# saidwivedi/InteractVLM

Measured on AMD Instinct MI355X. Metric: images/sec end-to-end contact inference, higher is better.
Workload: dtype f16

## Files before the change

### include/ivlm_hip.h

```cpp
#ifndef IVLM_HIP_H
#define IVLM_HIP_H

#include <stddef.h>
#include <stdint.h>

#ifdef __cplusplus
extern "C" {
#endif

#define IVLM_OK 0
#define IVLM_ERR_INVALID_ARG (-1)
#define IVLM_ERR_WORKSPACE (-2)
#define IVLM_ERR_LAUNCH (-3)
#define IVLM_ERR_UNSUPPORTED (-4)

#define IVLM_F32 0
#define IVLM_BF16 1
#define IVLM_BF16_SPLIT 2
#define IVLM_F16 4
#define IVLM_F16_SPLIT 5
#define IVLM_FP8 3

#define IVLM_GEMM_A_F32 1
#define IVLM_GEMM_RES_F32 2
// ... 233 lines not shown
typedef struct {
    int embed_dim, depth, heads, grid, window, patch, img_size, out_chans, mlp_dim;
} ivlm_sam_cfg;
typedef struct {
    const void *patch_w, *patch_b, *pos_embed, *neck0_w, *neck1_w, *neck1_b, *neck2_w, *neck3_w, *neck3_b;
} ivlm_sam_head;
typedef struct {
    const void *norm1_w, *norm1_b, *qkv_w, *qkv_b, *rel_h, *rel_w, *rel_cat, *proj_w, *proj_b, *norm2_w, *norm2_b, *lin1_w, *lin1_b,
        *lin2_w, *lin2_b;
    int global_attn;
} ivlm_sam_block;
size_t ivlm_sam_encode_workspace_bytes(const ivlm_sam_cfg *cfg, int V);
int ivlm_sam_encode(const ivlm_sam_cfg *cfg, const ivlm_sam_head *head, const ivlm_sam_block *blocks_host, const void *images, int V,
                    float *embeddings_out, void *workspace, size_t workspace_bytes, ivlm_stream_t stream);
size_t ivlm_sam_encode_parity_workspace_bytes(const ivlm_sam_cfg *cfg, int V);
int ivlm_sam_encode_parity(const ivlm_sam_cfg *cfg, const ivlm_sam_head *head, const ivlm_sam_block *blocks_host, const void *images,
                           int V, float *embeddings_out, void *workspace, size_t workspace_bytes, ivlm_stream_t stream);
typedef struct {
    const void *lin1_w16, *lin2_w16;
} ivlm_sam_mlp_f16;
int ivlm_sam_encode_parity_f16mlp(const ivlm_sam_cfg *cfg, const ivlm_sam_head *head, const ivlm_sam_block *blocks_host,
                                  const ivlm_sam_mlp_f16 *mlp16_host, const void *images, int V, float *embeddings_out,
                                  void *workspace, size_t workspace_bytes, ivlm_stream_t stream);
typedef struct {
    const void *qkv_w16, *proj_w16, *lin1_w16, *lin2_w16, *qkv_b16, *rel_cat16;
} ivlm_sam_block_f16;
size_t ivlm_sam_encode_f16_workspace_bytes(const ivlm_sam_cfg *cfg, int V);
int ivlm_sam_encode_f16(const ivlm_sam_cfg *cfg, const ivlm_sam_head *head, const ivlm_sam_block *blocks_host,
                        const ivlm_sam_block_f16 *blocks16_host, const void *images, int V, float *embeddings_out, void *workspace,
                        size_t workspace_bytes, ivlm_stream_t stream);
int ivlm_bf16_to_f16(const void *src_bf16, void *dst_f16, int64_t n, ivlm_stream_t stream);

typedef struct {
    const void *w2, *b;
    int n, k;
} ivlm_lin;
typedef struct {
    ivlm_lin q, k, v, o;
} ivlm_dec_attn;
typedef struct {
    ivlm_dec_attn self_attn, t2i, i2t;
    const void *norm1_w, *norm1_b, *norm2_w, *norm2_b, *norm3_w, *norm3_b, *norm4_w, *norm4_b;
    ivlm_lin lin1, lin2;
} ivlm_dec_layer;
typedef struct {
    int C, heads, depth;
    const void *no_mask, *key_pe, *out_tokens;
    ivlm_dec_layer layers[4];
    ivlm_dec_attn final_attn;
    const void *norm_final_w, *norm_final_b, *up_ln_w, *up_ln_b;
    ivlm_lin up0, up1, hyper[3], iou[3];
} ivlm_sam_dec;
size_t ivlm_sam_decode_workspace_bytes(int V, int grid, int C, int n_text, int mlp_dim);
int ivlm_sam_decode(const ivlm_sam_dec *weights, int V, int grid, int n_text, const float *image_embeddings,
                    const float *text_embeds, float *low_res_out, float *iou_out, void *workspace, size_t workspace_bytes,
                    ivlm_stream_t stream);

int ivlm_gemm_splitk_choice(int M, int N, int K, int act, int has_rms);
int ivlm_stages_splitk_fused(int on);

int ivlm_gemv1_bf12(const float *x, const void *P, int64_t ldp, const void *E, int64_t lde, const int32_t *ebase,
                    const int32_t *patch_ptr, const int32_t *patch_col, const void *patch_val, void *C, const void *bias,
                    const void *residual, int N, int K, int act, int out_f32, const void *rms_w, float rms_eps, int flags,
                    ivlm_stream_t stream);
int ivlm_gemv1_bf12m(const float *x, const void *Pf, const void *Ef, const int32_t *ebase, const int32_t *patch_ptr,
                     const int32_t *patch_col, const void *patch_val, void *C, const void *bias, const void *residual, int N, int K,
                     int act, int out_f32, const void *rms_w, float rms_eps, int flags, ivlm_stream_t stream);
int ivlm_llama_decode_attn_parts(const float *qkv, int cache_dtype, void *kcache, void *vcache, int tmax, float *parts, int H, int D,
                                 int pos, const int32_t *pos_dev, float theta, float scale, const float *cos_tab, const float *sin_tab,
                                 ivlm_stream_t stream);
int ivlm_gemv1_bf12m_parts(const float *parts, int D, const void *Pf, const void *Ef, const int32_t *ebase, const int32_t *patch_ptr,
                           const int32_t *patch_col, const void *patch_val, void *C, const void *bias, const void *residual, int N, int K,
                           int act, int out_f32, int flags, ivlm_stream_t stream);
int ivlm_pack_bf12m_count(const void *w, int N_valid, int n_rows, int K, int32_t *ebase, int32_t *patch_ptr, ivlm_stream_t stream);
int ivlm_pack_bf12m_fill(const void *w, int N_valid, int n_rows, int K, const int32_t *ebase, const int32_t *patch_ptr, void *Pf, void *Ef,
                         int32_t *patch_col, void *patch_val, ivlm_stream_t stream);
int ivlm_gemv16_bf12m(const float *x, int64_t lda, int M, const void *Pf, const void *Ef, const int32_t *ebase,
                      const int32_t *patch_ptr, const int32_t *patch_col, const void *patch_val, void *C, int64_t ldc, const void *bias,
                      const void *residual, int64_t ldr, int N, int K, int act, int out_f32, const void *rms_w, float rms_eps, int flags,
                      ivlm_stream_t stream);
void ivlm_gemv16_bf12m_tuning(int tiles_per_block);
int ivlm_decode_parts_tuning(int ranges);
void ivlm_gemv1_bf12m_tuning(int wide_max_blocks);
int ivlm_unpack_bf12(const void *P, int64_t ldp, const void *E, int64_t lde, const int32_t *ebase, const int32_t *patch_ptr,
                     const int32_t *patch_col, const void *patch_val, int N, int K, void *w_out, ivlm_stream_t stream);

int ivlm_argmax_f32(const float *x, int rows, int cols, int32_t *out, ivlm_stream_t stream);
int ivlm_argmax_f32_bump(const float *x, int rows, int cols, int32_t *out, int32_t *bump, ivlm_stream_t stream);

int ivlm_im2col_nchw(const void *x, void *out, int B, int C, int H, int W, int ks, int stride, int Kpad,
                     ivlm_stream_t stream);
int ivlm_im2col3x3_nhwc(const void *x, void *out, int B, int H, int W, int C, ivlm_stream_t stream);
int ivlm_im2col3x3_nhwc_strided(const void *x, int64_t ldx, void *out, int64_t ldo, int B, int H, int W, int C,
                                ivlm_stream_t stream);
int ivlm_gather_rows(void *dst, int dst_kind, int64_t ldd, const void *src, int src_dtype, int64_t lds, const int32_t *idx,
                     const void *add, int add_dtype, int64_t lda, int64_t rows, int cols, const float *fp8_scale,
                     ivlm_stream_t stream);
int ivlm_amax(const void *x, int dtype, int64_t n, float *out, ivlm_stream_t stream);
int ivlm_add_rows(void *out, int out_kind, const void *a, int a_dtype, const void *b, int b_dtype, int64_t rows, int cols,
                  int64_t b_rows, int op, ivlm_stream_t stream);
int ivlm_fill_rows(void *dst, int64_t ldd, const int32_t *idx, int64_t n_idx, const void *row, int cols,
                   ivlm_stream_t stream);
int ivlm_dense_pe(const void *gauss, void *pe, int pe_dtype, int h, int w, int F, ivlm_stream_t stream);
int ivlm_rope_kv(void *qkv, int64_t ld, int T, int H, int D, int pos0, float theta, void *kcache, void *vcache,
                 const float *cos_tab, const float *sin_tab, ivlm_stream_t stream);
int ivlm_rope_kv_f16(void *qkv, int64_t ld, int T, int H, int D, int pos0, float theta, void *kcache, void *vcache,
                     const float *cos_tab, const float *sin_tab, ivlm_stream_t stream);
int ivlm_rope_kv_split(void *qkv, int64_t ld, int T, int H, int D, int pos0, void *kcache, void *kcache_lo, void *vcache,
                       void *vcache_lo, const float *cos_tab, const float *sin_tab, ivlm_stream_t stream);
int ivlm_llama_attn_oproj(const float *qkv, void *kcache, void *vcache, int tmax, float *attn_scratch, const void *wo,
                          const float *x, float *x_out, int H, int D, float theta, float scale, const float *cos_tab,
                          const float *sin_tab, const int32_t *pos_dev, const int32_t *step_dev, int32_t *counter,
                          int32_t *status, ivlm_stream_t stream);
int ivlm_rope_table(float *cos_tab, float *sin_tab, int T, int D, float theta, ivlm_stream_t stream);
int ivlm_normalize_pad_u8(const uint8_t *src, int H, int W, int y0, int x0, int ch, int cw, const float *mean3_host,
                          const float *std3_host, void *out, int out_bf16, int OH, int OW, ivlm_stream_t stream);
int ivlm_mask_dot(const void *up, const void *hyper, int dtype, float *low, int B, int gh, int gw, int C,
                  ivlm_stream_t stream);

size_t ivlm_h_geo_workspace_bytes(int n);
int ivlm_h_geo_metric(const float *dist, const float *pred, const float *gt, int B, int n, float *out, void *workspace,
                      size_t workspace_bytes, ivlm_stream_t stream);
int ivlm_contact_prf(const float *gt, const float *pred, int B, int n, float thr, float *out, ivlm_stream_t stream);
int ivlm_spmv_csr(const int32_t *row_ptr, const int32_t *col, const float *val, const float *x, int B, int rows,
                  int cols, float *y, ivlm_stream_t stream);

int ivlm_contact_band_census(const float *p, int64_t ld, int B, int Nv, const float *thr, int J, float margin, int32_t *counts,
                             float *mindist, ivlm_stream_t stream);
size_t ivlm_mask_band_census_workspace_bytes(void);
int ivlm_mask_band_census(const float *logits, int V, int64_t HW, const int32_t *ent_pix, const int32_t *row_ptr, int n_rows,
                          float thr_p, float margin_p, int32_t *counts, void *workspace, size_t workspace_bytes,
                          ivlm_stream_t stream);

#define IVLM_SEG_GT_U8 0
#define IVLM_SEG_GT_I32 1
#define IVLM_SEG_GT_F32 2
size_t ivlm_seg_iou_workspace_bytes(int V);
int ivlm_seg_iou_counts(const float *pred, const void *gt, int gt_dtype, int V, int H, int W, int ignore_label, int32_t *out,
                        void *workspace, size_t workspace_bytes, ivlm_stream_t stream);
#define IVLM_AFFORD_MAX_N 4096
#define IVLM_AFFORD_MAX_T 64
int ivlm_afford_metrics(const float *gt, const float *pred, int B, int n, const float *thresholds, int T, float mae_div,
                        float *out, int32_t *valid, ivlm_stream_t stream);

#define IVLM_CONTACT_PAIR_CHAIN 512
size_t ivlm_contact_pair_workspace_bytes(int B, int N_o, int N_h);
int ivlm_contact_pair(const float *o, const float *h, const void *p, const void *q, int p_dtype, int B, int N_o, int N_h,
                      int64_t o_batch_stride, int64_t h_batch_stride, float *value_out, float *grad_o, float *grad_h,
                      void *workspace, size_t workspace_bytes, ivlm_stream_t stream);

#define IVLM_ICP_ESTIMATE_SCALE 1
#define IVLM_ICP_ALLOW_REFLECTION 2
#define IVLM_ICP_REQUERY 4
size_t ivlm_contact_icp_workspace_bytes(int B, int N_o);
int ivlm_contact_icp(const float *x, const float *y, const float *xn, const float *yn, const float *w, const float *init_R,
                     const float *init_T, const float *init_s, int B, int N_o, int N_h, int64_t x_batch_stride, int64_t y_batch_stride,
                     int64_t xn_batch_stride, int64_t yn_batch_stride, int64_t w_batch_stride, int max_iterations, float relative_rmse_thr,
                     int flags, float *R_out, float *T_out, float *s_out, float *rmse_out, int32_t *converged_out, int32_t *iterations_out,
                     int32_t *nn_idx_out, float *hist_R, float *hist_T, float *hist_s, void *workspace, size_t workspace_bytes,
                     ivlm_stream_t stream);

int ivlm_points_align(const float *X, const float *Y, const float *w, int B, int N, int64_t x_batch_stride, int64_t y_batch_stride,
                      int64_t w_batch_stride, int flags, float *R_out, float *T_out, float *s_out, void *workspace, size_t workspace_bytes,
                      ivlm_stream_t stream);

int ivlm_contact_nearest(const float *q, const float *t, int D, int B, int N_o, int N_h, int64_t q_batch_stride, int64_t t_batch_stride,
// ... 20 lines not shown
```

### interactvlm_amd/csrc/gemv_p12.hip

```cpp
#include <algorithm>

#include "kernels.h"

namespace ivlm {
namespace {

typedef __attribute__((ext_vector_type(4))) unsigned int u32x4_t;
typedef __attribute__((ext_vector_type(2))) unsigned int u32x2_t;
typedef __attribute__((ext_vector_type(4))) float f32x4v_t;

constexpr int kWaves = 16;
constexpr int kXScaleExp = 64;

struct P12 {
    const uint8_t* P;
    const uint8_t* E;
    int64_t ldp, lde;
    const int32_t* ebase;
    const int32_t* patch_ptr;
    const int32_t* patch_col;
    const bf16_t* patch_val;
};

template <int K>
// ... 69 lines not shown
        ssq = wave_sum(ssq);
        if (lane == 0) s_red[wave] = ssq;
    }
    __syncthreads();
    float acc = 0.0f;
    for (int c = lane; c < nw16; c += 64 * U) {
        if (c != lane) {
#pragma unroll
            for (int u = 0; u < U; ++u)
                if (c + 64 * u < nw16) {
                    w[u] = __builtin_nontemporal_load(pp + c + 64 * u);
                    e[u] = __builtin_nontemporal_load(ep + c + 64 * u);
                }
        }
#pragma unroll
        for (int u = 0; u < U; ++u) {
            const int cc = c + 64 * u;
            if (cc < nw16) {
                acc = dot4_p12(w[u][0], e[u][0], xf[2 * cc], acc);
                acc = dot4_p12(w[u][1], e[u][0] >> 16, xf[nchunk + 2 * cc], acc);
                acc = dot4_p12(w[u][2], e[u][1], xf[2 * cc + 1], acc);
                acc = dot4_p12(w[u][3], e[u][1] >> 16, xf[nchunk + 2 * cc + 1], acc);
            }
        }
    }
    float pacc = 0.0f;
    for (int i = p0 + lane; i < p1; i += 64) {
        const int col = p.patch_col[i];
        const int ch = col >> 3, wi = col & 7;
        const float xv = reinterpret_cast<const float*>(xf)[((wi < 4 ? ch : nchunk + ch) << 2) + (wi & 3)];
        pacc = fmaf(bf16_to_f32(p.patch_val[i]), xv, pacc);
    }
    acc = __builtin_ldexpf(wave_sum(acc), eb - kXScaleExp) + __builtin_ldexpf(wave_sum(pacc), -kXScaleExp);
    if (RMS) {
        float q = 0.0f;
#pragma unroll
        for (int i = 0; i < kWaves; ++i) q += s_red[i];
        acc *= rsqrtf(q / (float)g.K + g.rms_eps);
    }
    float v = acc + ((g.bias && live) ? bf16_to_f32(g.bias[row]) : 0.0f);
    if (g.act == ACT_SWIGLU) {
        if (lane == 0) s_val[wave] = v;
        __syncthreads();
        if (lane != 0 || (wave & 1) || !live) return;
        const float o = (v / (1.0f + __expf(-v))) * s_val[wave + 1];
        const int64_t idx = row >> 1;
        if (g.out_f32) static_cast<float*>(g.C)[idx] = o;
        else static_cast<bf16_t*>(g.C)[idx] = f32_to_bf16(o);
        return;
    }
    if (lane != 0 || !live) return;
    v = act1(v, g.act);
    if (g.residual) v += g.res_f32 ? reinterpret_cast<const float*>(g.residual)[row] : bf16_to_f32(g.residual[row]);
    if (g.out_f32) static_cast<float*>(g.C)[row] = v;
    else static_cast<bf16_t*>(g.C)[row] = f32_to_bf16(v);
}

struct P12M {
    const u32x4_t* P;
    const u32x2_t* E;
    const int32_t* ebase;
    const int32_t* patch_ptr;
    const int32_t* patch_col;
    const bf16_t* patch_val;
    const float* parts;
    int pD, pS;
};

typedef __attribute__((ext_vector_type(8))) __bf16 bf16x8m_t;
typedef __attribute__((ext_vector_type(4))) float f32x4m_t;

__device__ __forceinline__ uint32_t pair_p12m(uint32_t pd, uint32_t e) {
    return (pd & 0x807f807fu) | ((e * 0x00080080u) & 0x07800780u);
}
__device__ __forceinline__ bf16x8m_t frag_p12m(uint32_t x0, uint32_t x1, uint32_t e) {
    u32x4_t d;
    d[0] = pair_p12m(__builtin_amdgcn_perm(0u, x0, 0x01010000u), e & 0xffu);
    d[1] = pair_p12m(__builtin_amdgcn_perm(0u, x0, 0x03030202u), (e >> 8) & 0xffu);
    d[2] = pair_p12m(__builtin_amdgcn_perm(0u, x1, 0x01010000u), (e >> 16) & 0xffu);
    d[3] = pair_p12m(__builtin_amdgcn_perm(0u, x1, 0x03030202u), e >> 24);
    return __builtin_bit_cast(bf16x8m_t, d);
}

template <bool RMS, int kWavesM, int U, bool PARTS = false>
__global__ __launch_bounds__(64 * kWavesM, kWavesM == 16 ? 4 : 6) void gemv1_p12m_kernel(GemmArgs g, P12M p) {
    extern __shared__ __attribute__((aligned(16))) unsigned char smem[];
    __shared__ float s_red[kWavesM];
    __shared__ float s_part[kWavesM][16];
    __shared__ float s_patch[16];
    const int lane = threadIdx.x & 63, wave = __builtin_amdgcn_readfirstlane(threadIdx.x >> 6);
    const int K = g.K, nsp = K >> 6;
    const int per = (nsp + kWavesM - 1) / kWavesM;
    const int s0 = wave * per, s1 = min(nsp, s0 + per);
    const int64_t base = (int64_t)blockIdx.x * nsp * 64 + lane;
    const u32x4_t* pp = p.P + base;
    const u32x2_t* ep = p.E + base;
    u32x4_t w[U];
    u32x2_t e[U];
#pragma unroll
    for (int u = 0; u < U; ++u) {
        const int sp = min(s0 + u, nsp - 1);
        w[u] = __builtin_nontemporal_load(pp + (int64_t)sp * 64);
        e[u] = __builtin_nontemporal_load(ep + (int64_t)sp * 64);
    }
    constexpr bool EARLY = kWavesM == 16;
    const bool fin = wave == 0 && lane < 16;
    const int row = blockIdx.x * 16 + (lane & 15);
    int eb = 0;
    uint32_t bias_raw = 0, res_raw = 0;
    auto load_fin = [&]() {
        if (fin) {
            eb = p.ebase[row];
            if (g.bias) bias_raw = g.bias[row];
            if (g.residual) res_raw = g.res_f32 ? reinterpret_cast<const uint32_t*>(g.residual)[row] : (uint32_t)g.residual[row];
        }
    };
    int e_pp0 = 0, e_pp1 = 0, e_col = 0;
    uint32_t e_val = 0;
    if (EARLY) {
        e_pp0 = p.patch_ptr[blockIdx.x * 16 + wave];
        e_pp1 = p.patch_ptr[blockIdx.x * 16 + wave + 1];
        if (e_pp0 + lane < e_pp1) {
            e_col = p.patch_col[e_pp0 + lane];
            e_val = p.patch_val[e_pp0 + lane];
        }
        load_fin();
    }
    const float xs = __builtin_ldexpf(1.0f, kXScaleExp);
    float ssq = 0.0f;
    uint32_t* xw = reinterpret_cast<uint32_t*>(smem);
#ifdef IVLM_ABL_XSTAGE
    for (int c = threadIdx.x; c < (K >> 2) && !PARTS; c += 64 * kWavesM) {
        *reinterpret_cast<u32x2_t*>(xw + 2 * c) = u32x2_t{0x5f805f80u, 0x5f805f80u};
        *reinterpret_cast<u32x2_t*>(xw + (K >> 1) + 2 * c) = u32x2_t{0u, 0u};
        *reinterpret_cast<u32x2_t*>(xw + K + 2 * c) = u32x2_t{0u, 0u};
        ssq = 1.0f;
    }
    for (int c = threadIdx.x; c < (PARTS ? (K >> 2) : 0); c += 64 * kWavesM) {
#else
    for (int c = threadIdx.x; c < (K >> 2); c += 64 * kWavesM) {
#endif
        f32x4v_t xv4;
        if (PARTS) {
            const int k = c << 2, hd = k / p.pD, d0 = k - hd * p.pD, ps = p.pD + 4;
            const float* ph = p.parts + (int64_t)hd * p.pS * ps;
            float m[4], l[4];
            f32x4v_t o4[4];
#pragma unroll
            for (int s2 = 0; s2 < 4; ++s2) {
                const int sc = s2 < p.pS ? s2 : 0;
                m[s2] = ph[sc * ps + p.pD];
                l[s2] = ph[sc * ps + p.pD + 1];
                o4[s2] = *reinterpret_cast<const f32x4v_t*>(ph + sc * ps + d0);
            }
            const float M = fmaxf(fmaxf(m[0], m[1]), fmaxf(m[2], m[3]));
            float den = 0.0f;
            xv4 = f32x4v_t{0.0f, 0.0f, 0.0f, 0.0f};
#pragma unroll
            for (int s2 = 0; s2 < 4; ++s2) {
                const float wgt = s2 < p.pS ? __expf(m[s2] - M) : 0.0f;
                den = fmaf(wgt, l[s2], den);
                xv4 += o4[s2] * wgt;
            }
            xv4 = xv4 * (1.0f / den);
        } else {
            xv4 = reinterpret_cast<const f32x4v_t*>(g.A)[c];
        }
        float v[4] = {xv4[0], xv4[1], xv4[2], xv4[3]};
        if (RMS) {
            const u32x2_t gv = *(reinterpret_cast<const u32x2_t*>(g.rms_w) + c);
#pragma unroll
            for (int j = 0; j < 4; ++j) ssq += v[j] * v[j];
            v[0] *= __uint_as_float(gv[0] << 16);
            v[1] *= __uint_as_float(gv[0] & 0xffff0000u);
            v[2] *= __uint_as_float(gv[1] << 16);
            v[3] *= __uint_as_float(gv[1] & 0xffff0000u);
        }
        uint32_t hi[2], lo[2], l2[2];
#pragma unroll
        for (int j = 0; j < 2; ++j) {
            float a = v[2 * j] * xs, b = v[2 * j + 1] * xs;
            const float ah = bf16_to_f32(f32_to_bf16(a)), bh = bf16_to_f32(f32_to_bf16(b));
            hi[j] = pack_bf16x2(ah, bh);
            a -= ah;
            b -= bh;
            const float al = bf16_to_f32(f32_to_bf16(a)), bl = bf16_to_f32(f32_to_bf16(b));
            lo[j] = pack_bf16x2(al, bl);
            l2[j] = pack_bf16x2(a - al, b - bl);
        }
        *reinterpret_cast<u32x2_t*>(xw + 2 * c) = u32x2_t{hi[0], hi[1]};
        *reinterpret_cast<u32x2_t*>(xw + (K >> 1) + 2 * c) = u32x2_t{lo[0], lo[1]};
        *reinterpret_cast<u32x2_t*>(xw + K + 2 * c) = u32x2_t{l2[0], l2[1]};
    }
    if (RMS) {
        ssq = wave_sum(ssq);
        if (lane == 0) s_red[wave] = ssq;
    }
    __syncthreads();
    const int plane = min(lane & 15, 2);
    const u32x4_t* xa = reinterpret_cast<const u32x4_t*>(smem) + ((plane * K) >> 3) + (lane >> 4);
    f32x4m_t d = {0.0f, 0.0f, 0.0f, 0.0f};
    auto step_pair = [&](const u32x4_t& pw, const u32x2_t& ew, int sp) {
        const bf16x8m_t a0 = __builtin_bit_cast(bf16x8m_t, xa[sp * 8]);
        const bf16x8m_t a1 = __builtin_bit_cast(bf16x8m_t, xa[sp * 8 + 4]);
        d = __builtin_amdgcn_mfma_f32_16x16x32_bf16(a0, frag_p12m(pw[0], pw[1], ew[0]), d, 0, 0, 0);
        d = __builtin_amdgcn_mfma_f32_16x16x32_bf16(a1, frag_p12m(pw[2], pw[3], ew[1]), d, 0, 0, 0);
    };
    constexpr int UH = U / 2;
    for (int sp = s0; sp < s1; sp += U) {
#pragma unroll
        for (int hf = 0; hf < 2; ++hf) {
#pragma unroll
            for (int u = hf * UH; u < (hf + 1) * UH; ++u)
                if (sp + u < s1) step_pair(w[u], e[u], sp + u);
#pragma unroll
            for (int u = hf * UH; u < (hf + 1) * UH; ++u) {
                const int nx = sp + U + u;
                if (nx < s1) {
                    w[u] = __builtin_nontemporal_load(pp + (int64_t)nx * 64);
                    e[u] = __builtin_nontemporal_load(ep + (int64_t)nx * 64);
                }
            }
        }
    }
    if (lane < 16) s_part[wave][lane] = d[0] + d[1] + d[2];
    if (!EARLY) load_fin();
    if (EARLY) {
        asm volatile("" : "+v"(e_col), "+v"(e_val), "+v"(eb), "+v"(bias_raw), "+v"(res_raw));
    }
    const bf16_t* xb = reinterpret_cast<const bf16_t*>(smem);
    auto xat = [&](int col) { return (bf16_to_f32(xb[col]) + bf16_to_f32(xb[K + col])) + bf16_to_f32(xb[2 * K + col]); };
#pragma unroll
    for (int h = 0; h < 16 / kWavesM; ++h) {
        const int r = wave + kWavesM * h;
        const int pp0 = EARLY ? e_pp0 : p.patch_ptr[blockIdx.x * 16 + r];
        const int pp1 = EARLY ? e_pp1 : p.patch_ptr[blockIdx.x * 16 + r + 1];
        float pacc = 0.0f;
        if (pp0 < pp1) {
            int i = pp0 + lane;
            if (EARLY) {
                if (i < pp1) pacc = __uint_as_float(e_val << 16) * xat(e_col);
                i += 64;
            }
            for (; i < pp1; i += 64) pacc = fmaf(bf16_to_f32(p.patch_val[i]), xat(p.patch_col[i]), pacc);
            pacc = wave_sum(pacc);
        }
        if (lane == 0) s_patch[r] = pacc;
    }
    __syncthreads();
    if (!fin) return;
    float acc = 0.0f;
#pragma unroll
    for (int i = 0; i < kWavesM; ++i) acc += s_part[i][lane];
    acc = __builtin_ldexpf(acc, eb - kXScaleExp) + __builtin_ldexpf(s_patch[lane], -kXScaleExp);
    if (RMS) {
        float q = 0.0f;
#pragma unroll
        for (int i = 0; i < kWavesM; ++i) q += s_red[i];
        acc *= rsqrtf(q / (float)K + g.rms_eps);
    }
    float v = acc + __uint_as_float(bias_raw << 16);
    if (g.act == ACT_SWIGLU) {
        const float up = __shfl_down(v, 1, 64);
        if (lane & 1) return;
        const float o = (v / (1.0f + __expf(-v))) * up;
        const int64_t idx = row >> 1;
        if (g.out_f32) static_cast<float*>(g.C)[idx] = o;
        else static_cast<bf16_t*>(g.C)[idx] = f32_to_bf16(o);
        return;
    }
    v = act1(v, g.act) + __uint_as_float(g.res_f32 ? res_raw : res_raw << 16);
    if (g.out_f32) static_cast<float*>(g.C)[row] = v;
    else static_cast<bf16_t*>(g.C)[row] = f32_to_bf16(v);
}

__device__ __forceinline__ void split_pair_p12(float a, float b, uint32_t& hi, uint32_t& lo) {
    hi = pack_bf16x2(a, b);
    lo = pack_bf16x2(a - __uint_as_float(hi << 16), b - __uint_as_float(hi & 0xffff0000u));
}

template <bool RMS, int T>
__global__ __launch_bounds__(512, 2) void skinny_p12m_kernel(GemmArgs g, P12M p) {
    constexpr int kW = 8, U = 2;
    __shared__ float s_part[kW][16][17];
    __shared__ float s_ssq[kW][16];
    __shared__ float s_fin[16][17];
    const int lane = threadIdx.x & 63, wave = threadIdx.x >> 6;
    const int r = lane & 15, kg = lane >> 4;
    const int K = g.K, nsp = K >> 6;
    const int per = (nsp + kW - 1) / kW;
    const int s0 = wave * per, s1 = min(nsp, s0 + per);
    const int ntiles = g.N >> 4;
    const u32x4_t* pp[T];
    const u32x2_t* ep[T];
#pragma unroll
    for (int t = 0; t < T; ++t) {
        const int64_t rb = min((int)blockIdx.x * T + t, ntiles - 1);
        pp[t] = p.P + rb * nsp * 64 + lane;
        ep[t] = p.E + rb * nsp * 64 + lane;
    }
    const bool xrow = r < g.M;
    const u32x4_t* xp = reinterpret_cast<const u32x4_t*>(reinterpret_cast<const float*>(g.A) + (int64_t)(xrow ? r : 0) * g.lda);
    const u32x4_t* gp = reinterpret_cast<const u32x4_t*>(g.rms_w);
    const u32x4_t zero = {0u, 0u, 0u, 0u};
    const float xs = __builtin_ldexpf(1.0f, kXScaleExp);
    f32x4m_t acc[T];
#pragma unroll
    for (int t = 0; t < T; ++t) acc[t] = f32x4m_t{0.0f, 0.0f, 0.0f, 0.0f};
// ... 115 lines not shown
    for (int64_t i = (int64_t)blockIdx.x * 256 + threadIdx.x; i < total; i += (int64_t)gridDim.x * 256) {
        const int r = (int)(i / K), c = (int)(i - (int64_t)r * K);
        const uint32_t b = p.P[(int64_t)r * p.ldp + c];
        const uint32_t code = (p.E[(int64_t)r * p.lde + (c >> 1)] >> ((c & 1) * 4)) & 0xfu;
        out[i] = code ? (bf16_t)(((b & 0x80u) << 8) | ((uint32_t)(p.ebase[r] + (int)code) << 7) | (b & 0x7fu)) : (bf16_t)0;
    }
}
__global__ __launch_bounds__(256) void unpack_p12_patch_kernel(P12 p, int N, int K, bf16_t* __restrict__ out) {
    const int r = blockIdx.x;
    for (int i = p.patch_ptr[r] + threadIdx.x; i < p.patch_ptr[r + 1]; i += 256) out[(int64_t)r * K + p.patch_col[i]] = p.patch_val[i];
}

}
}

using namespace ivlm;

static bool p12_ok(const void* P, int64_t ldp, const void* E, int64_t lde, const int32_t* ebase, const int32_t* patch_ptr,
                   const int32_t* patch_col, const void* patch_val, int N, int K) {
    return P && E && ebase && patch_ptr && patch_col && patch_val && N > 0 && K > 0 && !(K & 15) && ldp >= K && lde >= K / 2 &&
           !(ldp & 15) && !(lde & 7) && !(reinterpret_cast<uintptr_t>(P) & 15) && !(reinterpret_cast<uintptr_t>(E) & 7);
}

extern "C" int ivlm_gemv1_bf12(const float* x, const void* P, int64_t ldp, const void* E, int64_t lde, const int32_t* ebase,
                               const int32_t* patch_ptr, const int32_t* patch_col, const void* patch_val, void* C, const void* bias,
                               const void* residual, int N, int K, int act, int out_f32, const void* rms_w, float rms_eps, int flags,
                               ivlm_stream_t stream) {
    ivlm_enter();
    if (!x || !C || !p12_ok(P, ldp, E, lde, ebase, patch_ptr, patch_col, patch_val, N, K)) return IVLM_ERR_INVALID_ARG;
    if ((size_t)K * 4 > 60 * 1024) return IVLM_ERR_UNSUPPORTED;
    if (act == ACT_SWIGLU && ((N & 1) || residual)) return IVLM_ERR_UNSUPPORTED;
    GemmArgs g;
    g.A = reinterpret_cast<const bf16_t*>(x);
    g.a_f32 = 1;
    g.C = C;
    g.bias = static_cast<const bf16_t*>(bias);
    g.residual = static_cast<const bf16_t*>(residual);
    g.res_f32 = (flags & IVLM_GEMM_RES_F32) ? 1 : 0;
    g.M = 1; g.N = N; g.K = K;
    g.lda = K;
    g.act = act;
    g.out_f32 = out_f32;
    g.rms_w = static_cast<const bf16_t*>(rms_w);
    g.rms_eps = rms_eps;
    P12 p{static_cast<const uint8_t*>(P), static_cast<const uint8_t*>(E), ldp, lde, ebase, patch_ptr, patch_col,
          static_cast<const bf16_t*>(patch_val)};
    hipStream_t st = ivlm_stream(stream);
    static ivlm_dev_mask_t set0{0}, set1{0};
    const dim3 grid((N + kWaves - 1) / kWaves), block(64 * kWaves);
    if (rms_w) {
        auto kfn = gemv1_p12_kernel<true>;
        if (ivlm_dev_pending(set1)) {
            (void)hipFuncSetAttribute(reinterpret_cast<const void*>(kfn), hipFuncAttributeMaxDynamicSharedMemorySize, 64 * 1024);
            ivlm_dev_done(set1);
        }
        ivlm_launch(kfn, grid, block, (size_t)K * 4, st, g, p);
    } else {
        auto kfn = gemv1_p12_kernel<false>;
        if (ivlm_dev_pending(set0)) {
            (void)hipFuncSetAttribute(reinterpret_cast<const void*>(kfn), hipFuncAttributeMaxDynamicSharedMemorySize, 64 * 1024);
            ivlm_dev_done(set0);
        }
        ivlm_launch(kfn, grid, block, (size_t)K * 4, st, g, p);
    }
    return ivlm_launch_status();
}

extern "C" int ivlm_unpack_bf12(const void* P, int64_t ldp, const void* E, int64_t lde, const int32_t* ebase, const int32_t* patch_ptr,
                                const int32_t* patch_col, const void* patch_val, int N, int K, void* w_out, ivlm_stream_t stream) {
    ivlm_enter();
    if (!w_out || !p12_ok(P, ldp, E, lde, ebase, patch_ptr, patch_col, patch_val, N, K)) return IVLM_ERR_INVALID_ARG;
    P12 p{static_cast<const uint8_t*>(P), static_cast<const uint8_t*>(E), ldp, lde, ebase, patch_ptr, patch_col,
          static_cast<const bf16_t*>(patch_val)};
    hipStream_t st = ivlm_stream(stream);
    const int64_t total = (int64_t)N * K;
    unpack_p12_kernel<<<(unsigned)std::min<int64_t>((total + 255) / 256, 65535 * 8), 256, 0, st>>>(p, N, K, static_cast<bf16_t*>(w_out));
    unpack_p12_patch_kernel<<<N, 256, 0, st>>>(p, N, K, static_cast<bf16_t*>(w_out));
    return ivlm_launch_status();
}

int g_skinny_p12m_tiles = 0;
int g_p12m_wide_max_blocks = 256;
int g_p12m_deep = 1;
namespace ivlm {
int g_decode_parts_S = 4;
}

static int gemv1_bf12m(const float* x, const float* parts, int pD, const void* Pf, const void* Ef, const int32_t* ebase,
                      const int32_t* patch_ptr, const int32_t* patch_col, const void* patch_val, void* C, const void* bias,
                      const void* residual, int N, int K, int act, int out_f32, const void* rms_w, float rms_eps, int flags,
                      ivlm_stream_t stream) {
    ivlm_enter();
    if ((!x && !parts) || !C || !Pf || !Ef || !ebase || !patch_ptr || !patch_col || !patch_val || N <= 0 || K <= 0)
        return IVLM_ERR_INVALID_ARG;
    if ((reinterpret_cast<uintptr_t>(Pf) & 15) || (reinterpret_cast<uintptr_t>(Ef) & 7) || (reinterpret_cast<uintptr_t>(x) & 15) ||
        (reinterpret_cast<uintptr_t>(parts) & 15))
        return IVLM_ERR_INVALID_ARG;
    if (parts && (pD <= 0 || (pD & 3) || K % pD != 0 || rms_w)) return IVLM_ERR_INVALID_ARG;
    if ((N & 15) || (K & 63) || (size_t)K * 6 > 100 * 1024) return IVLM_ERR_UNSUPPORTED;
    if (act == ACT_SWIGLU && residual) return IVLM_ERR_UNSUPPORTED;
    GemmArgs g;
    g.A = reinterpret_cast<const bf16_t*>(x);
    g.a_f32 = 1;
    g.C = C;
    g.bias = static_cast<const bf16_t*>(bias);
    g.residual = static_cast<const bf16_t*>(residual);
    g.res_f32 = (flags & IVLM_GEMM_RES_F32) ? 1 : 0;
    g.M = 1; g.N = N; g.K = K;
    g.lda = K;
    g.act = act;
    g.out_f32 = out_f32;
    g.rms_w = static_cast<const bf16_t*>(rms_w);
    g.rms_eps = rms_eps;
    P12M p{static_cast<const u32x4_t*>(Pf), static_cast<const u32x2_t*>(Ef), ebase, patch_ptr, patch_col,
           static_cast<const bf16_t*>(patch_val), parts, pD, g_decode_parts_S};
    hipStream_t st = ivlm_stream(stream);
    const dim3 grid(N / 16);
    const bool wide = grid.x <= (unsigned)g_p12m_wide_max_blocks;
    auto go = [&](auto kfn, int waves, ivlm_dev_mask_t& set) {
        if (ivlm_dev_pending(set)) {
            (void)hipFuncSetAttribute(reinterpret_cast<const void*>(kfn), hipFuncAttributeMaxDynamicSharedMemorySize, 100 * 1024);
            ivlm_dev_done(set);
        }
        ivlm_launch(kfn, grid, dim3(64 * waves), (size_t)K * 6, st, g, p);
    };
    static ivlm_dev_mask_t set[8];
    if (parts) {
        if (wide) go(gemv1_p12m_kernel<false, 16, 4, true>, 16, set[6]);
        else go(gemv1_p12m_kernel<false, 8, 4, true>, 8, set[7]);
        return ivlm_launch_status();
    }
    const bool deep = wide && (K >> 6) > 4 * 16 && g_p12m_deep;
    if (rms_w) {
        if (deep) go(gemv1_p12m_kernel<true, 16, 8>, 16, set[4]);
        else if (wide) go(gemv1_p12m_kernel<true, 16, 4>, 16, set[0]);
        else go(gemv1_p12m_kernel<true, 8, 4>, 8, set[1]);
    } else {
        if (deep) go(gemv1_p12m_kernel<false, 16, 8>, 16, set[5]);
        else if (wide) go(gemv1_p12m_kernel<false, 16, 4>, 16, set[2]);
        else go(gemv1_p12m_kernel<false, 8, 4>, 8, set[3]);
    }
    return ivlm_launch_status();
}

extern "C" int ivlm_gemv1_bf12m(const float* x, const void* Pf, const void* Ef, const int32_t* ebase, const int32_t* patch_ptr,
                                const int32_t* patch_col, const void* patch_val, void* C, const void* bias, const void* residual, int N,
                                int K, int act, int out_f32, const void* rms_w, float rms_eps, int flags, ivlm_stream_t stream) {
    if (!x) return IVLM_ERR_INVALID_ARG;
    return gemv1_bf12m(x, nullptr, 0, Pf, Ef, ebase, patch_ptr, patch_col, patch_val, C, bias, residual, N, K, act, out_f32, rms_w, rms_eps,
                       flags, stream);
}

extern "C" int ivlm_gemv1_bf12m_parts(const float* parts, int D, const void* Pf, const void* Ef, const int32_t* ebase,
                                      const int32_t* patch_ptr, const int32_t* patch_col, const void* patch_val, void* C, const void* bias,
                                      const void* residual, int N, int K, int act, int out_f32, int flags, ivlm_stream_t stream) {
    if (!parts) return IVLM_ERR_INVALID_ARG;
    return gemv1_bf12m(nullptr, parts, D, Pf, Ef, ebase, patch_ptr, patch_col, patch_val, C, bias, residual, N, K, act, out_f32, nullptr,
                       0.0f, flags, stream);
}

extern "C" void ivlm_gemv1_bf12m_tuning(int wide_max_blocks) {
    g_p12m_deep = wide_max_blocks >= 0;
    g_p12m_wide_max_blocks = wide_max_blocks < 0 ? -wide_max_blocks : wide_max_blocks;
}

extern "C" int ivlm_decode_parts_tuning(int ranges) {
    if (ranges != 2 && ranges != 4) return IVLM_ERR_INVALID_ARG;
    g_decode_parts_S = ranges;
    return IVLM_OK;
}

extern "C" int ivlm_gemv16_bf12m(const float* x, int64_t lda, int M, const void* Pf, const void* Ef, const int32_t* ebase,
                                 const int32_t* patch_ptr, const int32_t* patch_col, const void* patch_val, void* C, int64_t ldc,
                                 const void* bias, const void* residual, int64_t ldr, int N, int K, int act, int out_f32,
                                 const void* rms_w, float rms_eps, int flags, ivlm_stream_t stream) {
    ivlm_enter();
    if (!x || !C || !Pf || !Ef || !ebase || !patch_ptr || !patch_col || !patch_val || M <= 0 || M > 16 || N <= 0 || K <= 0)
        return IVLM_ERR_INVALID_ARG;
    if ((reinterpret_cast<uintptr_t>(Pf) & 15) || (reinterpret_cast<uintptr_t>(Ef) & 7) || (reinterpret_cast<uintptr_t>(x) & 15) ||
        (lda & 3) || lda < K)
        return IVLM_ERR_INVALID_ARG;
    if ((N & 15) || (K & 63)) return IVLM_ERR_UNSUPPORTED;
    if (act == ACT_SWIGLU && residual) return IVLM_ERR_UNSUPPORTED;
    if (ldc < (act == ACT_SWIGLU ? N / 2 : N) || (residual && ldr < N)) return IVLM_ERR_INVALID_ARG;
    GemmArgs g;
    g.A = reinterpret_cast<const bf16_t*>(x);
    g.a_f32 = 1;
    g.C = C;
    g.bias = static_cast<const bf16_t*>(bias);
    g.residual = static_cast<const bf16_t*>(residual);
    g.res_f32 = (flags & IVLM_GEMM_RES_F32) ? 1 : 0;
    g.M = M; g.N = N; g.K = K;
    g.lda = lda; g.ldc = ldc; g.ldr = ldr;
    g.act = act;
    g.out_f32 = out_f32;
    g.rms_w = static_cast<const bf16_t*>(rms_w);
    g.rms_eps = rms_eps;
    P12M p{static_cast<const u32x4_t*>(Pf), static_cast<const u32x2_t*>(Ef), ebase, patch_ptr, patch_col,
           static_cast<const bf16_t*>(patch_val), nullptr, 0, 0};
    hipStream_t st = ivlm_stream(stream);
    const int tiles = N / 16;
    int T = g_skinny_p12m_tiles;
    if (T <= 0) {
        int best_cost = 1 << 30;
        for (int t : {1, 2, 3}) {
            const int blocks = (tiles + t - 1) / t, cost = ((blocks + 255) / 256) * t;
            if (cost <= best_cost) { T = t; best_cost = cost; }
        }
    }
    const dim3 grid((tiles + T - 1) / T), block(512);
    if (rms_w) {
        if (T == 1) ivlm_launch(skinny_p12m_kernel<true, 1>, grid, block, 0, st, g, p);
        else if (T == 2) ivlm_launch(skinny_p12m_kernel<true, 2>, grid, block, 0, st, g, p);
        else ivlm_launch(skinny_p12m_kernel<true, 3>, grid, block, 0, st, g, p);
    } else {
        if (T == 1) ivlm_launch(skinny_p12m_kernel<false, 1>, grid, block, 0, st, g, p);
        else if (T == 2) ivlm_launch(skinny_p12m_kernel<false, 2>, grid, block, 0, st, g, p);
        else ivlm_launch(skinny_p12m_kernel<false, 3>, grid, block, 0, st, g, p);
    }
    return ivlm_launch_status();
}

extern "C" void ivlm_gemv16_bf12m_tuning(int tiles_per_block) { g_skinny_p12m_tiles = tiles_per_block > 3 ? 3 : tiles_per_block; }

namespace ivlm {
namespace {

__global__ __launch_bounds__(256) void p12_rowstats_kernel(const bf16_t* __restrict__ w, int n_valid, int K, int32_t* __restrict__ ebase,
                                                           int32_t* __restrict__ cnt) {
    __shared__ int s_red[4];
    const int row = blockIdx.x;
    int mx = 0;
    if (row < n_valid)
        for (int c = threadIdx.x; c < K; c += 256) mx = max(mx, (int)((w[(int64_t)row * K + c] >> 7) & 0xff));
    for (int o = 32; o; o >>= 1) mx = max(mx, __shfl_xor(mx, o, 64));
    if ((threadIdx.x & 63) == 0) s_red[threadIdx.x >> 6] = mx;
    __syncthreads();
    mx = max(max(s_red[0], s_red[1]), max(s_red[2], s_red[3]));
    const int eb = max(mx - 15, 0);
    int n = 0;
    if (row < n_valid)
        for (int c = threadIdx.x; c < K; c += 256) {
            const uint32_t b = w[(int64_t)row * K + c];
            n += ((int)((b >> 7) & 0xff) - eb < 1) && (b & 0x7fffu);
        }
    for (int o = 32; o; o >>= 1) n += __shfl_xor(n, o, 64);
// ... 107 lines not shown
```

Baseline: 10.52.

## Stage activation slices per wave to drop block barrier in gemv1 P12M kernel

For the wide 16-wave gemv1 variants without an RMSNorm prologue, each wave now stages only the activation chunks for its own K slice into shared memory. This lets the block-wide __syncthreads before the dot-product loop become a wavefront fence, with one barrier kept before the final reduction. The first few activation (or attention-part) loads are issued before the weight loads, separated by scheduling barriers, so their latency overlaps. The path is on by default and can be switched off with a new staging API. It adds template instantiations and makes correctness depend on each wave reading only the shared-memory chunks it wrote.

```diff
diff --git a/include/ivlm_hip.h b/include/ivlm_hip.h
--- a/include/ivlm_hip.h
+++ b/include/ivlm_hip.h
@@ -339,6 +339,7 @@
 void ivlm_gemv16_bf12m_tuning(int tiles_per_block);
 int ivlm_decode_parts_tuning(int ranges);
 void ivlm_gemv1_bf12m_tuning(int wide_max_blocks);
+int ivlm_gemv1_bf12m_staging(int form);
 int ivlm_unpack_bf12(const void *P, int64_t ldp, const void *E, int64_t lde, const int32_t *ebase, const int32_t *patch_ptr,
                      const int32_t *patch_col, const void *patch_val, int N, int K, void *w_out, ivlm_stream_t stream);
 
diff --git a/interactvlm_amd/csrc/gemv_p12.hip b/interactvlm_amd/csrc/gemv_p12.hip
--- a/interactvlm_amd/csrc/gemv_p12.hip
+++ b/interactvlm_amd/csrc/gemv_p12.hip
@@ -175,7 +175,7 @@
     return __builtin_bit_cast(bf16x8m_t, d);
 }
 
-template <bool RMS, int kWavesM, int U, bool PARTS = false>
+template <bool RMS, int kWavesM, int U, bool PARTS = false, bool WSTG = false>
 __global__ __launch_bounds__(64 * kWavesM, kWavesM == 16 ? 4 : 6) void gemv1_p12m_kernel(GemmArgs g, P12M p) {
     extern __shared__ __attribute__((aligned(16))) unsigned char smem[];
     __shared__ float s_red[kWavesM];
@@ -188,6 +188,50 @@
     const int64_t base = (int64_t)blockIdx.x * nsp * 64 + lane;
     const u32x4_t* pp = p.P + base;
     const u32x2_t* ep = p.E + base;
+    static_assert(!WSTG || (!RMS && kWavesM == 16), "per-wave staging: the 16-wave forms without RMSNorm prologue");
+    constexpr int kXEarly = !WSTG ? 0 : PARTS ? 1 : 4;
+    constexpr int kXE = kXEarly ? kXEarly : 1;
+    const int nch = K >> 2;
+    const int cw0 = s0 * 16 + lane, cw1 = s1 * 16;
+    const f32x4v_t* xg4 = reinterpret_cast<const f32x4v_t*>(g.A);
+    const u32x2_t* gg2 = reinterpret_cast<const u32x2_t*>(g.rms_w);
+    f32x4v_t xq[kXE], oq[PARTS ? kXE : 1][4];
+    u32x2_t mlq[PARTS ? kXE : 1][4];
+    auto load_parts = [&](int c, u32x2_t* ml, f32x4v_t* o4) {
+        const unsigned pd = p.pD;
+        const int k = c << 2, hd = (pd & (pd - 1)) ? (int)((unsigned)k / pd) : k >> __builtin_ctz(pd), d0 = k - hd * p.pD, ps = p.pD + 4;
+        const float* ph = p.parts + (int64_t)hd * p.pS * ps;
+#pragma unroll
+        for (int s2 = 0; s2 < 4; ++s2) {
+            const int sc = s2 < p.pS ? s2 : 0;
+            ml[s2] = *reinterpret_cast<const u32x2_t*>(ph + sc * ps + p.pD);
+            o4[s2] = *reinterpret_cast<const f32x4v_t*>(ph + sc * ps + d0);
+        }
+    };
+    if (WSTG) {
+#pragma unroll
+        for (int i = 0; i < kXEarly; ++i) {
+            const int c = cw0 + 64 * i;
+            xq[i] = f32x4v_t{0.0f, 0.0f, 0.0f, 0.0f};
+            if (PARTS) {
+#pragma unroll
+                for (int s2 = 0; s2 < 4; ++s2) {
+                    mlq[i][s2] = u32x2_t{0u, 0u};
+                    oq[i][s2] = f32x4v_t{0.0f, 0.0f, 0.0f, 0.0f};
+                }
+            }
+            if (c < cw1) {
+                if (PARTS) {
+                    load_parts(c, mlq[i], oq[i]);
+                } else {
+#ifndef IVLM_ABL_XSTAGE
+                    xq[i] = xg4[c];
+#endif
+                }
+            }
+        }
+        __builtin_amdgcn_sched_barrier(0);
+    }
     u32x4_t w[U];
     u32x2_t e[U];
 #pragma unroll
@@ -219,51 +263,36 @@
         }
         load_fin();
     }
+    if (WSTG) __builtin_amdgcn_sched_barrier(0);
     const float xs = __builtin_ldexpf(1.0f, kXScaleExp);
     float ssq = 0.0f;
     uint32_t* xw = reinterpret_cast<uint32_t*>(smem);
-#ifdef IVLM_ABL_XSTAGE
-    for (int c = threadIdx.x; c < (K >> 2) && !PARTS; c += 64 * kWavesM) {
-        *reinterpret_cast<u32x2_t*>(xw + 2 * c) = u32x2_t{0x5f805f80u, 0x5f805f80u};
-        *reinterpret_cast<u32x2_t*>(xw + (K >> 1) + 2 * c) = u32x2_t{0u, 0u};
-        *reinterpret_cast<u32x2_t*>(xw + K + 2 * c) = u32x2_t{0u, 0u};
-        ssq = 1.0f;
-    }
-    for (int c = threadIdx.x; c < (PARTS ? (K >> 2) : 0); c += 64 * kWavesM) {
-#else
-    for (int c = threadIdx.x; c < (K >> 2); c += 64 * kWavesM) {
-#endif
-        f32x4v_t xv4;
-        if (PARTS) {
-            const int k = c << 2, hd = k / p.pD, d0 = k - hd * p.pD, ps = p.pD + 4;
-            const float* ph = p.parts + (int64_t)hd * p.pS * ps;
-            float m[4], l[4];
-            f32x4v_t o4[4];
-#pragma unroll
-            for (int s2 = 0; s2 < 4; ++s2) {
-                const int sc = s2 < p.pS ? s2 : 0;
-                m[s2] = ph[sc * ps + p.pD];
-                l[s2] = ph[sc * ps + p.pD + 1];
-                o4[s2] = *reinterpret_cast<const f32x4v_t*>(ph + sc * ps + d0);
-            }
-            const float M = fmaxf(fmaxf(m[0], m[1]), fmaxf(m[2], m[3]));
-            float den = 0.0f;
-            xv4 = f32x4v_t{0.0f, 0.0f, 0.0f, 0.0f};
-#pragma unroll
-            for (int s2 = 0; s2 < 4; ++s2) {
-                const float wgt = s2 < p.pS ? __expf(m[s2] - M) : 0.0f;
-                den = fmaf(wgt, l[s2], den);
-                xv4 += o4[s2] * wgt;
-            }
-            xv4 = xv4 * (1.0f / den);
-        } else {
-            xv4 = reinterpret_cast<const f32x4v_t*>(g.A)[c];
-        }
+    auto merge_parts = [&](const u32x2_t* ml, const f32x4v_t* o4) {
+        float m[4], l[4];
+#pragma unroll
+        for (int s2 = 0; s2 < 4; ++s2) {
+            m[s2] = __uint_as_float(ml[s2][0]);
+            l[s2] = __uint_as_float(ml[s2][1]);
+        }
+        const float M = fmaxf(fmaxf(m[0], m[1]), fmaxf(m[2], m[3]));
+        float den = 0.0f;
+        f32x4v_t xv4 = {0.0f, 0.0f, 0.0f, 0.0f};
+#pragma unroll
+        for (int s2 = 0; s2 < 4; ++s2) {
+            const float wgt = s2 < p.pS ? __expf(m[s2] - M) : 0.0f;
+            den = fmaf(wgt, l[s2], den);
+            xv4 += o4[s2] * wgt;
+        }
+        return xv4 * (1.0f / den);
+    };
+    auto sum_squares = [&](const f32x4v_t& xv4) {
+        const float v[4] = {xv4[0], xv4[1], xv4[2], xv4[3]};
+#pragma unroll
+        for (int j = 0; j < 4; ++j) ssq += v[j] * v[j];
+    };
+    auto stage = [&](int c, const f32x4v_t& xv4, const u32x2_t& gv) {
         float v[4] = {xv4[0], xv4[1], xv4[2], xv4[3]};
         if (RMS) {
-            const u32x2_t gv = *(reinterpret_cast<const u32x2_t*>(g.rms_w) + c);
-#pragma unroll
-            for (int j = 0; j < 4; ++j) ssq += v[j] * v[j];
             v[0] *= __uint_as_float(gv[0] << 16);
             v[1] *= __uint_as_float(gv[0] & 0xffff0000u);
             v[2] *= __uint_as_float(gv[1] << 16);
@@ -284,12 +313,66 @@
         *reinterpret_cast<u32x2_t*>(xw + 2 * c) = u32x2_t{hi[0], hi[1]};
         *reinterpret_cast<u32x2_t*>(xw + (K >> 1) + 2 * c) = u32x2_t{lo[0], lo[1]};
         *reinterpret_cast<u32x2_t*>(xw + K + 2 * c) = u32x2_t{l2[0], l2[1]};
+    };
+#ifdef IVLM_ABL_XSTAGE
+    auto stage_const = [&](int c) {
+        *reinterpret_cast<u32x2_t*>(xw + 2 * c) = u32x2_t{0x5f805f80u, 0x5f805f80u};
+        *reinterpret_cast<u32x2_t*>(xw + (K >> 1) + 2 * c) = u32x2_t{0u, 0u};
+        *reinterpret_cast<u32x2_t*>(xw + K + 2 * c) = u32x2_t{0u, 0u};
+        ssq = 1.0f;
+    };
+    constexpr bool ABL = !PARTS;
+#else
+    auto stage_const = [&](int) {};
+    constexpr bool ABL = false;
+#endif
+    if (ABL) {
+        if (WSTG) {
+            for (int c = cw0; c < cw1; c += 64) stage_const(c);
+        } else {
+            for (int c = threadIdx.x; c < nch; c += 64 * kWavesM) stage_const(c);
+        }
+    } else if (WSTG) {
+        const u32x2_t no_gamma = {0u, 0u};
+#pragma unroll
+        for (int i = 0; i < kXEarly; ++i) {
+            const int c = cw0 + 64 * i;
+            if (c < cw1) stage(c, PARTS ? merge_parts(mlq[i], oq[i]) : xq[i], no_gamma);
+        }
+        for (int c = cw0 + 64 * kXEarly; c < cw1; c += 64) {
+            u32x2_t ml[4];
+            f32x4v_t o4[4], xv4;
+            if (PARTS) {
+                load_parts(c, ml, o4);
+                xv4 = merge_parts(ml, o4);
+            } else {
+                xv4 = xg4[c];
+            }
+            stage(c, xv4, no_gamma);
+        }
+    } else {
+        for (int c = threadIdx.x; c < nch; c += 64 * kWavesM) {
+            u32x2_t ml[4], gv = {0u, 0u};
+            f32x4v_t o4[4], xv4;
+            if (PARTS) {
+                load_parts(c, ml, o4);
+                xv4 = merge_parts(ml, o4);
+            } else {
+                xv4 = xg4[c];
+            }
+            if (RMS) {
+                gv = gg2[c];
+                sum_squares(xv4);
+            }
+            stage(c, xv4, gv);
+        }
     }
     if (RMS) {
         ssq = wave_sum(ssq);
         if (lane == 0) s_red[wave] = ssq;
     }
-    __syncthreads();
+    if (WSTG) __builtin_amdgcn_fence(__ATOMIC_ACQ_REL, "wavefront");
+    else __syncthreads();
     const int plane = min(lane & 15, 2);
     const u32x4_t* xa = reinterpret_cast<const u32x4_t*>(smem) + ((plane * K) >> 3) + (lane >> 4);
     f32x4m_t d = {0.0f, 0.0f, 0.0f, 0.0f};
@@ -317,6 +400,7 @@
         }
     }
     if (lane < 16) s_part[wave][lane] = d[0] + d[1] + d[2];
+    if (WSTG) __syncthreads();
     if (!EARLY) load_fin();
     if (EARLY) {
         asm volatile("" : "+v"(e_col), "+v"(e_val), "+v"(eb), "+v"(bias_raw), "+v"(res_raw));
@@ -598,6 +682,7 @@
 int g_skinny_p12m_tiles = 0;
 int g_p12m_wide_max_blocks = 256;
 int g_p12m_deep = 1;
+int g_p12m_staging = 1;
 namespace ivlm {
 int g_decode_parts_S = 4;
 }
@@ -640,21 +725,26 @@
         }
         ivlm_launch(kfn, grid, dim3(64 * waves), (size_t)K * 6, st, g, p);
     };
-    static ivlm_dev_mask_t set[8];
+    static ivlm_dev_mask_t set[11];
+    const bool wstg = g_p12m_staging && wide && !rms_w;
     if (parts) {
-        if (wide) go(gemv1_p12m_kernel<false, 16, 4, true>, 16, set[6]);
-        else go(gemv1_p12m_kernel<false, 8, 4, true>, 8, set[7]);
+        if (wstg) go(gemv1_p12m_kernel<false, 16, 4, true, true>, 16, set[8]);
+        else if (wide) go(gemv1_p12m_kernel<false, 16, 4, true, false>, 16, set[6]);
+        else go(gemv1_p12m_kernel<false, 8, 4, true, false>, 8, set[7]);
         return ivlm_launch_status();
     }
     const bool deep = wide && (K >> 6) > 4 * 16 && g_p12m_deep;
     if (rms_w) {
-        if (deep) go(gemv1_p12m_kernel<true, 16, 8>, 16, set[4]);
-        else if (wide) go(gemv1_p12m_kernel<true, 16, 4>, 16, set[0]);
-        else go(gemv1_p12m_kernel<true, 8, 4>, 8, set[1]);
+        if (deep) go(gemv1_p12m_kernel<true, 16, 8, false, false>, 16, set[4]);
+        else if (wide) go(gemv1_p12m_kernel<true, 16, 4, false, false>, 16, set[0]);
+        else go(gemv1_p12m_kernel<true, 8, 4, false, false>, 8, set[1]);
+    } else if (wstg) {
+        if (deep) go(gemv1_p12m_kernel<false, 16, 8, false, true>, 16, set[9]);
+        else go(gemv1_p12m_kernel<false, 16, 4, false, true>, 16, set[10]);
     } else {
-        if (deep) go(gemv1_p12m_kernel<false, 16, 8>, 16, set[5]);
-        else if (wide) go(gemv1_p12m_kernel<false, 16, 4>, 16, set[2]);
-        else go(gemv1_p12m_kernel<false, 8, 4>, 8, set[3]);
+        if (deep) go(gemv1_p12m_kernel<false, 16, 8, false, false>, 16, set[5]);
+        else if (wide) go(gemv1_p12m_kernel<false, 16, 4, false, false>, 16, set[2]);
+        else go(gemv1_p12m_kernel<false, 8, 4, false, false>, 8, set[3]);
     }
     return ivlm_launch_status();
 }
@@ -678,6 +768,12 @@
 extern "C" void ivlm_gemv1_bf12m_tuning(int wide_max_blocks) {
     g_p12m_deep = wide_max_blocks >= 0;
     g_p12m_wide_max_blocks = wide_max_blocks < 0 ? -wide_max_blocks : wide_max_blocks;
+}
+
+extern "C" int ivlm_gemv1_bf12m_staging(int form) {
+    if (form != 0 && form != 1) return IVLM_ERR_INVALID_ARG;
+    g_p12m_staging = form;
+    return IVLM_OK;
 }
 
 extern "C" int ivlm_decode_parts_tuning(int ranges) {
```

Result: faster. 10.69, median of 6 (+1.6%).
